# dmMaze/comic-text-detector

Hardware: AMD Instinct MI355X
Metric: pages/sec at 1024x1024 bs=32 (end-to-end detector, device-resident pages) (higher is better)
Workload: dtype f16

## Files before the change

comic-text-detector_amd/csrc/host_refine.cpp:

```cpp
#include <algorithm>
#include <cmath>
#include <cstdint>
#include <cstring>

#include "../../include/ctd_hip.h"
#include "host_refine.h"
#include "np_dispatch.h"

extern "C" int ctd_topk_colors(const int64_t* hist, double* colors) {
  int lo = -1, hi = -1;
  for (int v = 0; v < 256; ++v)
    if (hist[v] > 0) {
      if (lo < 0) lo = v;
      hi = v;
    }
  double first, last;
  if (lo < 0) first = 0.0, last = 1.0;
  else first = (double)lo, last = (double)hi;
  if (first == last) first -= 0.5, last += 0.5;
  const int nb = 255;
  double edges[256];
  const double step = (last - first) / (double)nb;
  for (int i = 0; i <= nb; ++i) edges[i] = (double)i * step + first;
  edges[nb] = last;
// ... 81 lines not shown
      const double c_top = std::min(top[k] + 30, 255.0);
      const double c_bottom = c_top - 60;
      rules[k].kind = 0;
      ctd_inrange_bounds(c_bottom, c_top, &rules[k].lo, &rules[k].hi);
    }
  }
  for (int ch = 0; ch < 3; ++ch) {
    for (int v = 0; v < 256; ++v) h[v] = hist4[256 * (1 + ch) + v];
    rules[3 + ch].kind = 1 + ch;
    rules[3 + ch].lo = ctd_otsu_from_hist(h);
    rules[3 + ch].hi = 0;
  }
}

int refine_candidates(const RRule rules[6], const uint64_t sums[6], long long npix, RCand out[4]) {
  int n = 0;
  auto pick = [&](int k) {
    RCand c;
    const unsigned long long d_pos = sums[k], d_neg = 255ull * (unsigned long long)npix - d_pos;
    c.rule = k;
    c.invert = d_neg < d_pos;
    c.dist = c.invert ? d_neg : d_pos;
    return c;
  };
  for (int k = 0; k < 3; ++k)
    if (rules[k].kind >= 0) out[n++] = pick(k);
  RCand best = pick(3);
  for (int k = 4; k < 6; ++k) {
    const RCand c = pick(k);
    if (c.dist < best.dist) best = c;
  }
  out[n++] = best;
  std::stable_sort(out, out + n, [](const RCand& a, const RCand& b) { return a.dist < b.dist; });
  return n;
}
```

comic-text-detector_amd/csrc/host_refine.h:

```cpp
#pragma once
#include <stdint.h>

struct RRule {
  int32_t kind;
  int32_t lo, hi;
};
struct RCand {
  int rule;
  int invert;
  unsigned long long dist;
};
void refine_rules(const uint32_t* hist4 , RRule rules[6]);
int refine_candidates(const RRule rules[6], const uint64_t sums[6], long long npix, RCand out[4]);
```

comic-text-detector_amd/csrc/kernels_twlds.hip:

```cpp
#include <algorithm>

#include "kernels.h"
#include "tail.h"

namespace {

constexpr int TL_MAXT = 1024;

struct Geo {
  int W, H, wp, words;
  unsigned last;
};

__device__ __forceinline__ unsigned lds_ld(const unsigned* p) {
  return __hip_atomic_load(p, __ATOMIC_RELAXED, __HIP_MEMORY_SCOPE_WORKGROUP);
}
__device__ __forceinline__ void lds_st(unsigned* p, unsigned v) {
  __hip_atomic_store(p, v, __ATOMIC_RELAXED, __HIP_MEMORY_SCOPE_WORKGROUP);
}

struct Row3 {
  unsigned prev, cur, nxt;
};
__device__ __forceinline__ Row3 row3(const unsigned* p, const Geo& g, int y, int wi) {
// ... 55 lines not shown
}
__device__ __forceinline__ void uf_union(unsigned* parent, unsigned a, unsigned b) {
  for (;;) {
    a = uf_find(parent, a);
    b = uf_find(parent, b);
    if (a == b) return;
    if (a < b) {
      const unsigned t = a;
      a = b;
      b = t;
    }
    if (atomicCAS(parent + a, a, b) == a) return;
  }
}

struct TLdsArgs {
  const TWin* wins;
  const TBand* bands;
  const int* order;
  int dilate;
  int max_words, rlay;
  int rcap;
  int* ovf;
};

__global__ __launch_bounds__(TL_MAXT) void tw_lds_kernel(TLdsArgs a) {
  extern __shared__ __attribute__((aligned(16))) unsigned lds[];
  const int t = threadIdx.x, lane = t & 63, wave = t >> 6;
  const int TL_NT = blockDim.x, NWV = TL_NT >> 6;
  const int widx = a.order[blockIdx.x];
  const TWin w = a.wins[widx];
  Geo g;
  g.W = w.w, g.H = w.h, g.wp = (w.w + 31) >> 5, g.words = g.wp * g.H;
  g.last = (w.w & 31) ? ((1u << (w.w & 31)) - 1u) : 0xffffffffu;
  const int MW = a.max_words, RL = a.rlay, RC = a.rcap;
  unsigned* const pred = lds;
  unsigned* const merged = lds + MW;
  unsigned* const cand = lds + 2 * MW;
  unsigned short* const base = (unsigned short*)(lds + 3 * MW);
  unsigned* const parent = lds + 3 * MW + ((MW + 1) >> 1);
  int* const acc = (int*)(parent + RL);
  unsigned* const red = parent + 2 * RL;
  unsigned* const tmp = parent;
  auto validw = [&](int wi) { return wi == g.wp - 1 ? g.last : 0xffffffffu; };
  const int y_t = t / g.wp, wi_t = t - y_t * g.wp;
  const int dy_t = TL_NT / g.wp, dwi_t = TL_NT - dy_t * g.wp;
  auto for_words = [&](auto&& fn) {
    int y = y_t, wi = wi_t;
    for (int i = t; i < g.words; i += TL_NT) {
      fn(i, y, wi);
      wi += dwi_t, y += dy_t;
      if (wi >= g.wp) wi -= g.wp, ++y;
    }
  };

  for_words([&](int i, int y, int wi) {
    unsigned v[8];
    load32(w.mask + (size_t)(w.y1 + y) * w.mask_w + w.x1 + 32 * wi, g.W - 32 * wi, v);
    unsigned bits = 0;
#pragma unroll
    for (int j = 0; j < 8; ++j) bits |= gt60_nibble(v[j]) << (4 * j);
    tmp[i] = bits & validw(wi);
    merged[i] = 0;
  });
  __syncthreads();
  for_words([&](int i, int y, int wi) {
    auto ext = [&](int yy, int ww) -> unsigned {
      if ((unsigned)yy >= (unsigned)g.H || (unsigned)ww >= (unsigned)g.wp) return 0xffffffffu;
      return tmp[yy * g.wp + ww] | ~validw(ww);
    };
    const unsigned cur = ext(y, wi), prev = ext(y, wi - 1), nxt = ext(y, wi + 1);
    pred[i] = cur & ((cur << 1) | (prev >> 31)) & ((cur >> 1) | (nxt << 31)) & ext(y - 1, wi) & ext(y + 1, wi) & validw(wi);
  });
  __syncthreads();

  const int seg = (g.words + TL_NT - 1) / TL_NT;
  auto starts_of = [&](int i, int wi) -> unsigned {
    const unsigned c = cand[i], cl = wi > 0 ? cand[i - 1] : 0u;
    return c & ~((c << 1) | (cl >> 31));
  };
  auto scan_runs = [&]() -> int {
    const int i0 = min(t * seg, g.words), i1 = min(i0 + seg, g.words);
    int cnt = 0;
    {
      int wi = i0 % g.wp;
      for (int i = i0; i < i1; ++i) {
        cnt += __popc(starts_of(i, wi));
        if (++wi == g.wp) wi = 0;
      }
// ... 79 lines not shown
    for_words([&](int i, int, int wi) {
      const unsigned c = cand[i];
      if (!c) return;
      const unsigned cl = wi > 0 ? cand[i - 1] : 0u;
      const unsigned sc = c & ~((c << 1) | (cl >> 31)), bc = base[i];
      unsigned add = 0;
      for_groups(c, [&](int p, unsigned grp) {
        if (acc[uf_find(parent, rid_from(bc, sc, p))] > 0) add |= grp;
      });
      if (add) merged[i] |= add;
    });
    __syncthreads();
  };
  bool overflow = false;

  for (int r = 0; r < w.nband && !overflow; ++r) {
    const TBand bd = a.bands[w.band0 + r];
    for_words([&](int i, int y, int wi) {
      const int npx = min(32, g.W - 32 * wi);
      const uint8_t* src = w.img + ((size_t)(w.y1 + y) * w.img_w + w.x1 + 32 * wi) * 3;
      unsigned v[24];
      load32(src, min(32, 3 * npx), v);
      load32(src + 32, min(32, max(0, 3 * npx - 32)), v + 8);
      load32(src + 64, min(32, max(0, 3 * npx - 64)), v + 16);
      unsigned bits = 0;
      auto byte_at = [&](int o) { return (v[o >> 2] >> (8 * (o & 3))) & 0xffu; };
      if (bd.kind == 0) {
#pragma unroll
        for (int k = 0; k < 32; ++k) {
          const int gr = gray3(byte_at(3 * k), byte_at(3 * k + 1), byte_at(3 * k + 2));
          bits |= ((gr >= bd.lo && gr <= bd.hi) ? 1u : 0u) << k;
        }
      } else {
        const int ch = bd.kind - 1;
#pragma unroll
        for (int k = 0; k < 32; ++k) {
          const unsigned c0 = byte_at(3 * k), c1 = byte_at(3 * k + 1), c2 = byte_at(3 * k + 2);
          bits |= (((int)(ch == 0 ? c0 : (ch == 1 ? c1 : c2)) > bd.lo) ? 1u : 0u) << k;
        }
      }
      if (bd.invert) bits = ~bits;
      tmp[i] = bits & validw(wi);
    });
    __syncthreads();
    for_words([&](int i, int y, int wi) {
      const Row3 c0 = row3(tmp, g, y, wi);
      unsigned out = c0.cur;
      if (out) {
        const Row3 m1 = row3(tmp, g, y - 1, wi), p1 = row3(tmp, g, y + 1, wi), m2 = row3(tmp, g, y - 2, wi), p2 = row3(tmp, g, y + 2, wi);
        const unsigned up = ring3(m1), dn = ring3(p1), cur = c0.cur;
        const unsigned single = cur & ~(shk<-1>(c0) | shk<1>(c0) | up | dn);
        const unsigned hl = cur & shk<1>(c0) & ~(shk<-1>(c0) | shk<2>(c0) | up | dn | shk<2>(m1) | shk<2>(p1));
        const unsigned hr = cur & shk<-1>(c0) & ~(shk<-2>(c0) | shk<1>(c0) | up | dn | shk<-2>(m1) | shk<-2>(p1));
        const unsigned vt = cur & p1.cur & ~(shk<-1>(c0) | shk<1>(c0) | shk<-1>(p1) | shk<1>(p1) | up | ring3(p2));
        const unsigned vb = cur & m1.cur & ~(shk<-1>(c0) | shk<1>(c0) | shk<-1>(m1) | shk<1>(m1) | dn | ring3(m2));
        out = cur & ~(single | hl | hr | vt | vb);
      }
      cand[i] = out;
// ... 103 lines not shown
      if ((unsigned)v2) atomicOr(ap, (unsigned)v2);
      if ((unsigned)(v2 >> 32)) atomicOr(ap + 1, (unsigned)(v2 >> 32));
    }
  });
}

}

size_t tw_lds_bytes(int max_words, int rcap) {
  const int rlay = std::max(rcap, (max_words + 1) / 2);
  return ((size_t)3 * max_words + (max_words + 1) / 2 + (size_t)2 * rlay + 20) * 4;
}

int tw_lds_rcap(int max_words) { return std::min(65000, std::max(1024, (int)((long long)max_words * g_tw_lds_runs_x10 / 10))); }

bool launch_tw_lds(const TWin* wins, const TBand* bands, const int* order, int n, int max_words, int rcap, int dilate, int* ovf,
                   hipStream_t st, TwLdsLaunch* used) {
  if (n <= 0) return true;
  TLdsArgs a;
  a.wins = wins, a.bands = bands, a.order = order, a.dilate = dilate, a.max_words = max_words;
  a.rcap = std::min(rcap, 65000), a.rlay = std::max(a.rcap, (max_words + 1) / 2);
  a.ovf = ovf;
  const size_t bytes = tw_lds_bytes(max_words, a.rcap);
  const int nt = g_tw_lds_threads >= 1024 ? 1024 : (g_tw_lds_threads >= 512 ? 512 : 256);
  if (used) *used = TwLdsLaunch{n, max_words, a.rcap, nt, (int)bytes, 0};
  if (bytes > 48 * 1024 &&
      hipFuncSetAttribute((const void*)tw_lds_kernel, hipFuncAttributeMaxDynamicSharedMemorySize, (int)bytes) != hipSuccess) {
    (void)hipGetLastError();
    if (used) used->refused = 1;
    return false;
  }
  hipLaunchKernelGGL(tw_lds_kernel, dim3(n), dim3(nt), bytes, st, a);
  return true;
}
```

comic-text-detector_amd/csrc/tail.h:

```cpp
#pragma once
#include "ctd_common.h"
#include "tuning.h"

struct DbcTables {
  int B, H, W, cap, rcap;
  const float* prob;
  long long prob_stride;
  const int* lab;
  const int* n_f;
  const int* n_b;
  const int* st_f;
  const int* st_b;
  const int* first_f;
  const int* first_b;
  int* par_f;
  int* par_b;
  int* off_f;
  int* off_b;
  int* hdr;
  int* row_lo;
  int* row_hi;
  double* sum_f;
  double* sum_b;
  double* ring_sum;
// ... 32 lines not shown
void launch_tw_accept_all(const TWin* wins, const TBand* bands, int n, const int* labels, int canvas_w, const int* stats,
                          int max_labels, int min_box, uint8_t* merged, int merged_w, unsigned* counters, hipStream_t st);
void launch_tw_dilate(const TWin* wins, int n, int max_pix, const uint8_t* in, uint8_t* out, uint8_t* comp, int merged_w,
                      unsigned* count255, int dilate, hipStream_t st);
void launch_tw_holes(const TWin* wins, int n, int max_pix, const int* labels2, const int* stats2, const int* first2,
                     int max_labels, const unsigned* count255, int* top2, uint8_t* merged, int merged_w,
                     unsigned* counters2, hipStream_t st);
void launch_tw_holes_all(const TWin* wins, int n, const int* labels2, const int* stats2, const int* first2, int max_labels,
                         const unsigned* count255, uint8_t* merged, int merged_w, unsigned* counters2, hipStream_t st);
void launch_tw_commit(const TWin* wins, int n, int max_pix, const uint8_t* merged, int merged_w, hipStream_t st);
size_t tw_lds_bytes(int max_words, int rcap);
int tw_lds_rcap(int max_words);
struct TwLdsLaunch {
  int n, max_words, rcap, threads, bytes, refused;
};
bool launch_tw_lds(const TWin* wins, const TBand* bands, const int* order, int n, int max_words, int rcap, int dilate, int* ovf,
                   hipStream_t st, TwLdsLaunch* used = nullptr);
void launch_mask_clear_where(uint8_t* mask, const uint8_t* refined, long long n, int thr, hipStream_t st);
void launch_copy2d_u8(const uint8_t* src, int spitch, uint8_t* dst, int dpitch, int rows, int cols, hipStream_t st);

struct MSeg {
  void* dst;
  const void* src;
  unsigned long long row_bytes;
  long long dpitch, spitch;
  int rows;
  int fill;
  int vec;
  int pad_;
};
constexpr int kMSegMax = 24;
struct MSegs {
// ... 6 lines not shown
```

comic-text-detector_amd/csrc/tail.hip:

```cpp
#include <algorithm>
#include <atomic>
#include <chrono>
#include <mutex>
#include <cmath>
#include <cstring>
#include <string>
#include <thread>
#include <vector>

#include "host_refine.h"
#include "kernels.h"
#include "tail.h"

int ctd_fail_msg(int code, const std::string& msg);

#define T_TRY(expr)                                                                                  \
  do {                                                                                               \
    hipError_t e_ = (expr);                                                                          \
    if (e_ != hipSuccess) return ctd_fail_msg(CTD_ERR_HIP, std::string(#expr) + ": " + hipGetErrorString(e_)); \
  } while (0)

namespace {

struct DevBuf {
// ... 184 lines not shown
}

static_assert(sizeof(ctd_trace_win) == 4312, "ctd_trace_win is read as a packed record (comic-text-detector_amd/tail.py)");
struct DbTrace {
  int32_t hdr[4] = {0, 0, 0, 0};
  int nf = 0, nb = 0, nr = 0;
  std::vector<int32_t> i32;
  std::vector<double> f64;
};

struct ctd_tail {
  int device = 0;
  hipStream_t st = nullptr;
  DevBuf d_dets, d_nms_ws, d_lab_f, d_ccl_ws, d_ccl_small, d_dbc_i, d_dbc_d, d_rows, d_pmask, d_refined;
  DevBuf d_wins, d_rules, d_bands, d_hist, d_sums, d_canvas, d_clab, d_cstats, d_cnt, d_merged, d_mlab, d_mstats, d_cnt2, d_small, d_crop;
  DevBuf d_wins_c, d_bands_c, d_lds;
  PinBuf h_dets, h_hdr, h_tab, h_pmask, h_refined, h_hist, h_sums, h_wins, h_rules, h_bands, h_small, h_lab;
  PinBuf h_wins_c, h_bands_c, h_lds;
  int B = 0;
  std::vector<ctd_tail_page> pages;
  std::vector<size_t> poff;
  std::vector<uint8_t*> hmask;
  size_t ptotal = 0;
  std::vector<PageOut> out;
  double ms_stage[10] = {0, 0, 0, 0, 0, 0, 0, 0, 0, 0};
  double ms_db_wait = 0;
  double ms_sub[5] = {0, 0, 0, 0, 0};
  int host_threads = 8;
  int n_lds = 0, n_canvas = 0, n_ovf = 0;
  long long lds_per_block = 64 << 10;
  double ms_lds_wait = 0;
  bool trace = false;
  std::vector<ctd_trace_win> tr_wins;
// ... 125 lines not shown
  launch_tw_dilate(dw, n, max_pix, merged_a, merged_b, comp, pm.W, count255, refine_mode == 0 ? 1 : 0, st);
  GET(t->d_mlab, mpx * 4, int, mlab);
  GET(t->d_mstats, (size_t)cap2 * 6 * 4, int, mstats);
  int* mfirst = mstats + (size_t)cap2 * 5;
  launch_ccl(comp, 1, pm.H, pm.W, 0, 8, mlab, n_dev, mstats, cap2, ws, st, 0, mfirst, 1);
  launch_label_counters_zero(counters2, n_dev, cap2, st);
  if (fused) launch_tw_holes_all(dw, n, mlab, mstats, mfirst, cap2, count255, merged_b, pm.W, counters2, st);
  else launch_tw_holes(dw, n, max_pix, mlab, mstats, mfirst, cap2, count255, top2, merged_b, pm.W, counters2, st);
  launch_tw_commit(dw, n, max_pix, merged_b, pm.W, st);
  T_TRY(chain.end());
  T_TRY(hipGetLastError());
  return CTD_OK;
}

void trace_windows(ctd_tail* t, const std::vector<WinReq>& reqs, int pass, const uint32_t* hhist, const RRule* hrules,
                   const uint64_t* hsums, const std::vector<int>& canvas_win, const std::vector<int>& again) {
  const size_t base = t->tr_wins.size();
  t->tr_wins.resize(base + reqs.size());
  for (size_t i = 0; i < reqs.size(); ++i) {
    ctd_trace_win& r = t->tr_wins[base + i];
    std::memset(&r, 0, sizeof(r));
    r.page = reqs[i].page, r.x1 = reqs[i].x1, r.y1 = reqs[i].y1, r.w = reqs[i].x2 - reqs[i].x1, r.h = reqs[i].y2 - reqs[i].y1;
    r.pass = pass, r.path = 0;
    std::memcpy(r.hist, hhist + i * 1024, sizeof(r.hist));
    for (int k = 0; k < 6; ++k) {
      const RRule& rl = hrules[i * 6 + k];
      r.rules[3 * k] = rl.kind, r.rules[3 * k + 1] = rl.lo, r.rules[3 * k + 2] = rl.hi;
      r.sums[k] = hsums[i * 6 + k];
    }
    RCand c[4];
    r.n_cand = refine_candidates(hrules + i * 6, hsums + i * 6, (long long)r.w * r.h, c);
    for (int k = 0; k < r.n_cand; ++k) r.cand_rule[k] = c[k].rule, r.cand_invert[k] = c[k].invert, r.cand_dist[k] = c[k].dist;
  }
  for (int i : canvas_win) t->tr_wins[base + i].path = 1;
  for (int i : again) t->tr_wins[base + i].path = 2;
}

int refine_windows(ctd_tail* t, const std::vector<WinReq>& reqs, int refine_mode, int pass) {
  const int n = (int)reqs.size();
  if (n == 0) return CTD_OK;
  hipStream_t st = t->st;
  GET(t->d_pmask, 0, uint8_t, pmask);
  GET(t->d_refined, 0, uint8_t, refined);
  std::vector<int> ww(n), wh(n);
  int max_pix = 1;
  for (int i = 0; i < n; ++i) {
    ww[i] = reqs[i].x2 - reqs[i].x1, wh[i] = reqs[i].y2 - reqs[i].y1;
// ... 2 lines not shown
  GET(t->h_wins, sizeof(TWin) * n, TWin, hw);
  for (int i = 0; i < n; ++i) {
    const ctd_tail_page& pg = t->pages[reqs[i].page];
    TWin& w = hw[i];
    w.img = pg.img_dev;
    w.mask = pmask + t->poff[reqs[i].page];
    w.out = refined + t->poff[reqs[i].page];
    w.img_w = pg.im_w, w.mask_w = pg.im_w, w.out_w = pg.im_w;
    w.x1 = reqs[i].x1, w.y1 = reqs[i].y1, w.w = ww[i], w.h = wh[i];
    w.mx = 0, w.my = 0;
    w.band0 = 0, w.nband = 0;
  }
  GET(t->d_wins, sizeof(TWin) * n, TWin, dw);
  GET(t->d_hist, (size_t)n * 1024 * 4, unsigned, dhist);
  GET(t->h_hist, (size_t)n * 1024 * 4, uint32_t, hhist);
  GET(t->d_sums, (size_t)n * 6 * 8, unsigned long long, dsums);
  GET(t->h_sums, (size_t)n * 6 * 8, uint64_t, hsums);
  Batch bt(st);
  T_TRY(bt.h2d(dw, hw, sizeof(TWin) * n));
  bt.fill(dhist, 0, (size_t)n * 1024 * 4);
  bt.fill(dsums, 0, (size_t)n * 6 * 8);
  bt.flush();
  launch_tw_hist(dw, n, max_pix, dhist, st);
  T_TRY(bt.d2h(hhist, dhist, (size_t)n * 1024 * 4));
  bt.flush();
  const double tr0 = now_ms();
  T_TRY(hipStreamSynchronize(st));
  const double tr1 = now_ms();
  GET(t->h_rules, sizeof(RRule) * 6 * n, RRule, hrules);
  parallel_for(n, t->host_threads, [&](int i) { refine_rules(hhist + (size_t)i * 1024, hrules + (size_t)i * 6); });
  static_assert(sizeof(RRule) == sizeof(TRule), "rule layouts must agree");
  GET(t->d_rules, sizeof(TRule) * 6 * n, TRule, drules);
  T_TRY(bt.h2d(drules, hrules, sizeof(TRule) * 6 * n));
  bt.flush();
  launch_tw_xor(dw, drules, n, max_pix, dsums, st);
  T_TRY(bt.d2h(hsums, dsums, (size_t)n * 6 * 8));
  bt.flush();
  const double tr2 = now_ms();
  T_TRY(hipStreamSynchronize(st));
  const double tr3 = now_ms();
  std::vector<TBand> bands;
  for (int i = 0; i < n; ++i) {
    RCand c[4];
    const int nc = refine_candidates(hrules + (size_t)i * 6, hsums + (size_t)i * 6, (long long)ww[i] * wh[i], c);
    hw[i].band0 = (int)bands.size(), hw[i].nband = nc;
    for (int r = 0; r < nc; ++r) {
      const RRule& rl = hrules[(size_t)i * 6 + c[r].rule];
      TBand b;
      b.win = i, b.cx = b.cy = 0, b.kind = rl.kind, b.lo = rl.lo, b.hi = rl.hi, b.invert = c[r].invert, b.round = r;
      bands.push_back(b);
    }
  }
  const int nbands = (int)bands.size();
  const long long lds_max = std::min(g_tail_lds_max_bytes, t->lds_per_block - 2048);
  std::vector<int> lds_win, canvas_win;
  std::vector<int> words(n);
  for (int i = 0; i < n; ++i) {
    words[i] = ((ww[i] + 31) >> 5) * wh[i];
    const int rc = g_tail_lds_rcap > 0 ? g_tail_lds_rcap : tw_lds_rcap(words[i]);
    if (g_tail_lds && (long long)tw_lds_bytes(words[i], std::max(rc, (words[i] + 1) / 2)) <= lds_max) lds_win.push_back(i);
    else canvas_win.push_back(i);
  }
  int nl = (int)lds_win.size();
  int* hovf = nullptr;
  if (nl) {
    std::stable_sort(lds_win.begin(), lds_win.end(), [&](int a, int b) { return words[a] < words[b]; });
    GET(t->h_bands, sizeof(TBand) * std::max(nbands, 1), TBand, hb);
    std::memcpy(hb, bands.data(), sizeof(TBand) * nbands);
    GET(t->d_bands, sizeof(TBand) * std::max(nbands, 1), TBand, db);
    GET(t->h_lds, (size_t)n * 8, int, hl);
    GET(t->d_lds, (size_t)n * 8, int, dl);
    std::memcpy(hl, lds_win.data(), sizeof(int) * nl);
    hovf = hl + n;
    T_TRY(bt.h2d(db, hb, sizeof(TBand) * nbands));
    T_TRY(bt.h2d(dw, hw, sizeof(TWin) * n));
    T_TRY(bt.h2d(dl, hl, sizeof(int) * nl));
    bt.fill(dl + n, 0, sizeof(int) * n);
    bt.flush();
    const long long cls[3] = {g_tail_lds_cls0, g_tail_lds_cls1, lds_max};
    std::vector<int> refused;
    int k0 = 0;
    for (int c = 0; c < 3 && k0 < nl; ++c) {
      int k1 = k0;
      auto need = [&](int k) {
        const int wd = words[lds_win[k]];
        const int rc = g_tail_lds_rcap > 0 ? g_tail_lds_rcap : tw_lds_rcap(wd);
        return (long long)tw_lds_bytes(wd, std::max(rc, (wd + 1) / 2));
      };
      while (k1 < nl && (c == 2 || need(k1) <= cls[c])) ++k1;
      if (k1 > k0) {
        const int mw = words[lds_win[k1 - 1]];
        TwLdsLaunch used{};
        if (!launch_tw_lds(dw, db, dl + k0, k1 - k0, mw, g_tail_lds_rcap > 0 ? g_tail_lds_rcap : tw_lds_rcap(mw),
                           refine_mode == 0 ? 1 : 0, dl + n, st, t->trace ? &used : nullptr))
          for (int k = k0; k < k1; ++k) refused.push_back(lds_win[k]);
        if (t->trace) t->tr_lds.push_back(used);
      }
      k0 = k1;
    }
    T_TRY(bt.d2h(hovf, dl + n, sizeof(int) * n));
    bt.flush();
    if (!refused.empty()) {
      std::sort(refused.begin(), refused.end());
      canvas_win.insert(canvas_win.end(), refused.begin(), refused.end());
      std::sort(canvas_win.begin(), canvas_win.end());
      std::vector<int> kept;
      for (int i : lds_win)
        if (!std::binary_search(refused.begin(), refused.end(), i)) kept.push_back(i);
      lds_win.swap(kept);
      nl = (int)lds_win.size();
    }
  }
  if (int rc = refine_canvas(t, hw, bands, canvas_win, refine_mode)) return rc;
  const double tr4 = now_ms();
  double tr5 = tr4;
  std::vector<int> again;
  if (nl) {
    T_TRY(hipStreamSynchronize(st));
    tr5 = now_ms();
    for (int k = 0; k < nl; ++k)
      if (hovf[lds_win[k]]) again.push_back(lds_win[k]);
    std::sort(again.begin(), again.end());
    t->n_lds += nl - (int)again.size(), t->n_canvas += (int)canvas_win.size() + (int)again.size(), t->n_ovf += (int)again.size();
    if (int rc = refine_canvas(t, hw, bands, again, refine_mode)) return rc;
  } else {
    t->n_canvas += (int)canvas_win.size();
  }
  T_TRY(hipGetLastError());
  if (t->trace) trace_windows(t, reqs, pass, hhist, hrules, hsums, canvas_win, again);
  t->ms_stage[4] += tr1 - tr0;
  t->ms_stage[5] += tr3 - tr2;
  t->ms_stage[6] += (now_ms() - tr5) + (tr4 - tr3) + (tr2 - tr1);
  t->ms_lds_wait += tr5 - tr4;
  return CTD_OK;
}

int layout_pages(ctd_tail* t, int B, const ctd_tail_page* pages) {
  t->B = B;
  t->pages.assign(pages, pages + B);
  t->poff.resize(B);
  size_t off = 0;
  for (int b = 0; b < B; ++b) {
    if (pages[b].im_h < 1 || pages[b].im_w < 1) return ctd_fail_msg(CTD_ERR_INVALID, "bad page size");
    t->poff[b] = off;
// ... 372 lines not shown
  if (hipDeviceGetAttribute(&smem, hipDeviceAttributeMaxSharedMemoryPerBlock, device) == hipSuccess && smem > 0) t->lds_per_block = smem;
  *out = t;
  return CTD_OK;
}

void ctd_tail_destroy(ctd_tail* t) {
  if (!t) return;
  (void)hipSetDevice(t->device);
  if (t->st) {
    (void)hipStreamSynchronize(t->st);
    (void)hipStreamDestroy(t->st);
  }
  DevBuf* dv[] = {&t->d_dets, &t->d_nms_ws, &t->d_lab_f, &t->d_ccl_ws, &t->d_ccl_small, &t->d_dbc_i, &t->d_dbc_d,
                  &t->d_rows, &t->d_pmask, &t->d_refined, &t->d_wins, &t->d_rules, &t->d_bands, &t->d_hist, &t->d_sums,
                  &t->d_canvas, &t->d_clab, &t->d_cstats, &t->d_cnt, &t->d_merged, &t->d_mlab, &t->d_mstats, &t->d_cnt2,
                  &t->d_small, &t->d_crop, &t->d_wins_c, &t->d_bands_c, &t->d_lds};
  for (DevBuf* d : dv) d->release();
  PinBuf* pv[] = {&t->h_dets, &t->h_hdr, &t->h_tab, &t->h_pmask, &t->h_refined, &t->h_hist, &t->h_sums, &t->h_wins,
                  &t->h_rules, &t->h_bands, &t->h_small, &t->h_lab, &t->h_wins_c, &t->h_bands_c, &t->h_lds};
  for (PinBuf* p : pv) p->release();
  delete t;
}

void* ctd_tail_stream(ctd_tail* t) { return t ? (void*)t->st : nullptr; }

static int drained(ctd_tail* t, int rc) {
  if (rc != CTD_OK && t && t->st) (void)hipStreamSynchronize(t->st);
  return rc;
}

static int tail_run_impl(ctd_tail* t, int32_t B, int32_t Hn, int32_t Wn, const float* blks_dev, int32_t rows, int32_t no,
                         const uint8_t* mask_u8_dev, const float* prob_dev, int64_t prob_stride, const uint8_t* bitmap_dev,
                         const ctd_tail_page* pages, const ctd_tail_params* prm, uint8_t* const* mask_out,
                         uint8_t* const* refined_out, void* ready_event) {
// ... 404 lines not shown
```

Before: 3255.

## Fuse refine-rule sums and candidate selection into the LDS window kernel

Result: no change. 3276 (median of 6 runs) (+0.6%).

```diff
diff --git a/comic-text-detector_amd/csrc/host_refine.cpp b/comic-text-detector_amd/csrc/host_refine.cpp
--- a/comic-text-detector_amd/csrc/host_refine.cpp
+++ b/comic-text-detector_amd/csrc/host_refine.cpp
@@ -119,23 +119,8 @@
 }
 
 int refine_candidates(const RRule rules[6], const uint64_t sums[6], long long npix, RCand out[4]) {
-  int n = 0;
-  auto pick = [&](int k) {
-    RCand c;
-    const unsigned long long d_pos = sums[k], d_neg = 255ull * (unsigned long long)npix - d_pos;
-    c.rule = k;
-    c.invert = d_neg < d_pos;
-    c.dist = c.invert ? d_neg : d_pos;
-    return c;
-  };
+  unsigned valid3 = 0;
   for (int k = 0; k < 3; ++k)
-    if (rules[k].kind >= 0) out[n++] = pick(k);
-  RCand best = pick(3);
-  for (int k = 4; k < 6; ++k) {
-    const RCand c = pick(k);
-    if (c.dist < best.dist) best = c;
-  }
-  out[n++] = best;
-  std::stable_sort(out, out + n, [](const RCand& a, const RCand& b) { return a.dist < b.dist; });
-  return n;
+    if (rules[k].kind >= 0) valid3 |= 1u << k;
+  return refine_decide(valid3, sums, npix, out);
 }
diff --git a/comic-text-detector_amd/csrc/host_refine.h b/comic-text-detector_amd/csrc/host_refine.h
--- a/comic-text-detector_amd/csrc/host_refine.h
+++ b/comic-text-detector_amd/csrc/host_refine.h
@@ -1,14 +1,7 @@
 #pragma once
 #include <stdint.h>
 
-struct RRule {
-  int32_t kind;
-  int32_t lo, hi;
-};
-struct RCand {
-  int rule;
-  int invert;
-  unsigned long long dist;
-};
+#include "refine_decide.h"
+
 void refine_rules(const uint32_t* hist4 , RRule rules[6]);
 int refine_candidates(const RRule rules[6], const uint64_t sums[6], long long npix, RCand out[4]);
diff --git a/comic-text-detector_amd/csrc/kernels_twlds.hip b/comic-text-detector_amd/csrc/kernels_twlds.hip
--- a/comic-text-detector_amd/csrc/kernels_twlds.hip
+++ b/comic-text-detector_amd/csrc/kernels_twlds.hip
@@ -1,6 +1,10 @@
 #include <algorithm>
 
+#include <mutex>
+#include <type_traits>
+
 #include "kernels.h"
+#include "refine_decide.h"
 #include "tail.h"
 
 namespace {
@@ -93,16 +97,48 @@
   }
 }
 
+template <int From, int To, class F>
+__device__ __forceinline__ void static_for(F&& f) {
+  if constexpr (From < To) {
+    f(std::integral_constant<int, From>{});
+    static_for<From + 1, To>(f);
+  }
+}
+
 struct TLdsArgs {
   const TWin* wins;
   const TBand* bands;
+  const TRule* rules;
   const int* order;
   int dilate;
   int max_words, rlay;
   int rcap;
   int* ovf;
+  unsigned long long* sums;
+  unsigned* cword;
 };
 
+struct GeK {
+  unsigned add, nd, en;
+};
+__device__ __forceinline__ GeK ge_const(int d) {
+  d = min(max(d, 0), 256);
+  GeK k;
+  k.en = d > 255 ? 0u : 0x80808080u;
+  k.add = (0x80u - (unsigned)(d & 0x7f)) * 0x01010101u;
+  k.nd = (d & 0x80) ? 0u : 0xffffffffu;
+  return k;
+}
+__device__ __forceinline__ unsigned ge4(unsigned x, const GeK& k) {
+  const unsigned t = (x & 0x7f7f7f7fu) + k.add;
+  return ((x & t) | ((x | t) & k.nd)) & k.en;
+}
+__device__ __forceinline__ unsigned gather4(unsigned w0, unsigned w1, unsigned w2, unsigned w3, int s) {
+  const unsigned sel = 0x0c0c0000u | ((4u + (unsigned)s) << 8) | (unsigned)s;
+  return __builtin_amdgcn_perm(w1, w0, sel) | (__builtin_amdgcn_perm(w3, w2, sel) << 16);
+}
+
+template <int WPT>
 __global__ __launch_bounds__(TL_MAXT) void tw_lds_kernel(TLdsArgs a) {
   extern __shared__ __attribute__((aligned(16))) unsigned lds[];
   const int t = threadIdx.x, lane = t & 63, wave = t >> 6;
@@ -132,17 +168,110 @@
       if (wi >= g.wp) wi -= g.wp, ++y;
     }
   };
-
-  for_words([&](int i, int y, int wi) {
-    unsigned v[8];
-    load32(w.mask + (size_t)(w.y1 + y) * w.mask_w + w.x1 + 32 * wi, g.W - 32 * wi, v);
-    unsigned bits = 0;
-#pragma unroll
-    for (int j = 0; j < 8; ++j) bits |= gt60_nibble(v[j]) << (4 * j);
-    tmp[i] = bits & validw(wi);
-    merged[i] = 0;
-  });
-  __syncthreads();
+  auto for_owned = [&](auto&& fn) {
+    int y = y_t, wi = wi_t;
+    static_for<0, WPT>([&](auto jc) {
+      const int i = t + decltype(jc)::value * TL_NT;
+      if (i < g.words) fn(jc, i, y, wi);
+      wi += dwi_t, y += dy_t;
+      if (wi >= g.wp) wi -= g.wp, ++y;
+    });
+  };
+  unsigned pl[WPT > 0 ? WPT : 1][6];
+  unsigned cw = 0;
+
+  if constexpr (WPT == 0) {
+    for_words([&](int i, int y, int wi) {
+      unsigned v[8];
+      load32(w.mask + (size_t)(w.y1 + y) * w.mask_w + w.x1 + 32 * wi, g.W - 32 * wi, v);
+      unsigned bits = 0;
+#pragma unroll
+      for (int j = 0; j < 8; ++j) bits |= gt60_nibble(v[j]) << (4 * j);
+      tmp[i] = bits & validw(wi);
+      merged[i] = 0;
+    });
+    __syncthreads();
+  } else {
+    GeK glo[3], ghi[3], gch[3];
+    int chn[3];
+    unsigned valid3 = 0, used6 = 0;
+#pragma unroll
+    for (int k = 0; k < 3; ++k) {
+      const TRule rg = a.rules[(size_t)widx * 6 + k], rc = a.rules[(size_t)widx * 6 + 3 + k];
+      const bool on = rg.kind == 0;
+      glo[k] = ge_const(on ? rg.lo : 256);
+      ghi[k] = ge_const(min(rg.hi, 255) + 1);
+      gch[k] = ge_const(rc.kind >= 1 ? min(rc.lo, 255) + 1 : 256);
+      chn[k] = rc.kind;
+      valid3 |= (rg.kind >= 0 ? 1u : 0u) << k;
+      used6 |= ((rg.kind >= 0 ? 1u : 0u) << k) | ((rc.kind >= 0 ? 1u : 0u) << (3 + k));
+    }
+    if (t < 13) red[t] = 0u;
+    unsigned cnt[6] = {0, 0, 0, 0, 0, 0}, msum[6] = {0, 0, 0, 0, 0, 0}, mall = 0;
+#pragma unroll
+    for (int j = 0; j < WPT; ++j)
+#pragma unroll
+      for (int k = 0; k < 6; ++k) pl[j][k] = 0u;
+    for_owned([&](auto jc, int i, int y, int wi) {
+      constexpr int j = decltype(jc)::value;
+      const int npx = min(32, g.W - 32 * wi);
+      const uint8_t* src = w.img + ((size_t)(w.y1 + y) * w.img_w + w.x1 + 32 * wi) * 3;
+      unsigned v[24], mv[8];
+      load32(w.mask + (size_t)(w.y1 + y) * w.mask_w + w.x1 + 32 * wi, npx, mv);
+      load32(src, min(32, 3 * npx), v);
+      load32(src + 32, min(32, max(0, 3 * npx - 32)), v + 8);
+      load32(src + 64, min(32, max(0, 3 * npx - 64)), v + 16);
+      unsigned bits = 0;
+#pragma unroll
+      for (int q = 0; q < 8; ++q) {
+        bits |= gt60_nibble(mv[q]) << (4 * q);
+        mall = __builtin_amdgcn_sad_u8(mv[q], 0u, mall);
+      }
+      tmp[i] = bits & validw(wi);
+      merged[i] = 0;
+      unsigned p6[6] = {0, 0, 0, 0, 0, 0};
+#pragma unroll
+      for (int q = 0; q < 8; ++q) {
+        const unsigned m4 = gather4(mv[q >> 2], mv[2 + (q >> 2)], mv[4 + (q >> 2)], mv[6 + (q >> 2)], q & 3);
+        unsigned c4[3];
+#pragma unroll
+        for (int c = 0; c < 3; ++c) {
+          const int o = 3 * q + c;
+          c4[c] = gather4(v[o >> 2], v[6 + (o >> 2)], v[12 + (o >> 2)], v[18 + (o >> 2)], o & 3);
+        }
+        unsigned y4 = 0;
+#pragma unroll
+        for (int k = 0; k < 4; ++k)
+          y4 |= (unsigned)gray3((c4[0] >> (8 * k)) & 0xffu, (c4[1] >> (8 * k)) & 0xffu, (c4[2] >> (8 * k)) & 0xffu) << (8 * k);
+#pragma unroll
+        for (int k = 0; k < 6; ++k) {
+          unsigned on;
+          if (k < 3) {
+            on = ge4(y4, glo[k]) & ~ge4(y4, ghi[k]);
+          } else {
+            const int ch = chn[k - 3];
+            on = ge4(ch == 1 ? c4[0] : (ch == 2 ? c4[1] : c4[2]), gch[k - 3]);
+          }
+          p6[k] |= on >> (7 - q);
+          msum[k] = __builtin_amdgcn_sad_u8(m4 & (on | (on - (on >> 7))), 0u, msum[k]);
+        }
+      }
+      const unsigned vw = validw(wi);
+#pragma unroll
+      for (int k = 0; k < 6; ++k) {
+        pl[j][k] = p6[k];
+        cnt[k] += (unsigned)__popc(p6[k] & vw);
+      }
+    });
+    __syncthreads();
+#pragma unroll
+    for (int k = 0; k < 13; ++k) {
+      unsigned x = k < 6 ? cnt[k] : (k < 12 ? msum[k - 6] : mall);
+      for (int off = 32; off > 0; off >>= 1) x += __shfl_down(x, off);
+      if (lane == 0 && x) atomicAdd(red + k, x);
+    }
+    cw = valid3 | (used6 << 8);
+  }
   for_words([&](int i, int y, int wi) {
     auto ext = [&](int yy, int ww) -> unsigned {
       if ((unsigned)yy >= (unsigned)g.H || (unsigned)ww >= (unsigned)g.wp) return 0xffffffffu;
@@ -152,6 +281,22 @@
     pred[i] = cur & ((cur << 1) | (prev >> 31)) & ((cur >> 1) | (nxt << 31)) & ext(y - 1, wi) & ext(y + 1, wi) & validw(wi);
   });
   __syncthreads();
+  if constexpr (WPT > 0) {
+    const unsigned valid3 = cw & 7u, used6 = cw >> 8;
+    const unsigned long long M = red[12];
+    uint64_t sums[6];
+#pragma unroll
+    for (int k = 0; k < 6; ++k)
+      sums[k] = ((used6 >> k) & 1u) ? 255ull * red[k] + M - 2ull * red[6 + k] : 0ull;
+    RCand cs[4];
+    const int nc = refine_decide(valid3, sums, (long long)g.W * g.H, cs);
+    cw = refine_pack(nc, cs);
+    if (t == 0) {
+#pragma unroll
+      for (int k = 0; k < 6; ++k) a.sums[(size_t)widx * 6 + k] = sums[k];
+      a.cword[widx] = cw;
+    }
+  }
 
   const int seg = (g.words + TL_NT - 1) / TL_NT;
   auto starts_of = [&](int i, int wi) -> unsigned {
@@ -261,34 +406,50 @@
   };
   bool overflow = false;
 
-  for (int r = 0; r < w.nband && !overflow; ++r) {
-    const TBand bd = a.bands[w.band0 + r];
-    for_words([&](int i, int y, int wi) {
-      const int npx = min(32, g.W - 32 * wi);
-      const uint8_t* src = w.img + ((size_t)(w.y1 + y) * w.img_w + w.x1 + 32 * wi) * 3;
-      unsigned v[24];
-      load32(src, min(32, 3 * npx), v);
-      load32(src + 32, min(32, max(0, 3 * npx - 32)), v + 8);
-      load32(src + 64, min(32, max(0, 3 * npx - 64)), v + 16);
-      unsigned bits = 0;
-      auto byte_at = [&](int o) { return (v[o >> 2] >> (8 * (o & 3))) & 0xffu; };
-      if (bd.kind == 0) {
-#pragma unroll
-        for (int k = 0; k < 32; ++k) {
-          const int gr = gray3(byte_at(3 * k), byte_at(3 * k + 1), byte_at(3 * k + 2));
-          bits |= ((gr >= bd.lo && gr <= bd.hi) ? 1u : 0u) << k;
+  const int nround = WPT > 0 ? refine_word_count(cw) : w.nband;
+  for (int r = 0; r < nround && !overflow; ++r) {
+    if constexpr (WPT > 0) {
+      const int rule = refine_word_rule(cw, r);
+      const unsigned inv = refine_word_invert(cw, r) ? 0xffffffffu : 0u;
+      unsigned pick[6];
+#pragma unroll
+      for (int k = 0; k < 6; ++k) pick[k] = rule == k ? 0xffffffffu : 0u;
+      for_owned([&](auto jc, int i, int, int wi) {
+        constexpr int j = decltype(jc)::value;
+        unsigned bits = 0;
+#pragma unroll
+        for (int k = 0; k < 6; ++k) bits |= pl[j][k] & pick[k];
+        tmp[i] = (bits ^ inv) & validw(wi);
+      });
+    } else {
+      const TBand bd = a.bands[w.band0 + r];
+      for_words([&](int i, int y, int wi) {
+        const int npx = min(32, g.W - 32 * wi);
+        const uint8_t* src = w.img + ((size_t)(w.y1 + y) * w.img_w + w.x1 + 32 * wi) * 3;
+        unsigned v[24];
+        load32(src, min(32, 3 * npx), v);
+        load32(src + 32, min(32, max(0, 3 * npx - 32)), v + 8);
+        load32(src + 64, min(32, max(0, 3 * npx - 64)), v + 16);
+        unsigned bits = 0;
+        auto byte_at = [&](int o) { return (v[o >> 2] >> (8 * (o & 3))) & 0xffu; };
+        if (bd.kind == 0) {
+#pragma unroll
+          for (int k = 0; k < 32; ++k) {
+            const int gr = gray3(byte_at(3 * k), byte_at(3 * k + 1), byte_at(3 * k + 2));
+            bits |= ((gr >= bd.lo && gr <= bd.hi) ? 1u : 0u) << k;
+          }
+        } else {
+          const int ch = bd.kind - 1;
+#pragma unroll
+          for (int k = 0; k < 32; ++k) {
+            const unsigned c0 = byte_at(3 * k), c1 = byte_at(3 * k + 1), c2 = byte_at(3 * k + 2);
+            bits |= (((int)(ch == 0 ? c0 : (ch == 1 ? c1 : c2)) > bd.lo) ? 1u : 0u) << k;
+          }
         }
-      } else {
-        const int ch = bd.kind - 1;
-#pragma unroll
-        for (int k = 0; k < 32; ++k) {
-          const unsigned c0 = byte_at(3 * k), c1 = byte_at(3 * k + 1), c2 = byte_at(3 * k + 2);
-          bits |= (((int)(ch == 0 ? c0 : (ch == 1 ? c1 : c2)) > bd.lo) ? 1u : 0u) << k;
-        }
-      }
-      if (bd.invert) bits = ~bits;
-      tmp[i] = bits & validw(wi);
-    });
+        if (bd.invert) bits = ~bits;
+        tmp[i] = bits & validw(wi);
+      });
+    }
     __syncthreads();
     for_words([&](int i, int y, int wi) {
       const Row3 c0 = row3(tmp, g, y, wi);
@@ -422,22 +583,59 @@
 
 int tw_lds_rcap(int max_words) { return std::min(65000, std::max(1024, (int)((long long)max_words * g_tw_lds_runs_x10 / 10))); }
 
-bool launch_tw_lds(const TWin* wins, const TBand* bands, const int* order, int n, int max_words, int rcap, int dilate, int* ovf,
-                   hipStream_t st, TwLdsLaunch* used) {
+namespace {
+
+int tw_lds_threads() { return g_tw_lds_threads >= 1024 ? 1024 : (g_tw_lds_threads >= 512 ? 512 : 256); }
+
+constexpr int kLdsDevices = 64;
+template <int WPT>
+hipError_t lds_limit_once() {
+  static std::once_flag once[kLdsDevices];
+  static hipError_t err[kLdsDevices];
+  int dev = 0;
+  if (hipError_t e = hipGetDevice(&dev)) return e;
+  if (dev < 0 || dev >= kLdsDevices) return hipErrorInvalidDevice;
+  std::call_once(once[dev], [&] {
+    int lim = 0;
+    hipError_t e = hipDeviceGetAttribute(&lim, hipDeviceAttributeMaxSharedMemoryPerBlock, dev);
+    if (e == hipSuccess) e = hipFuncSetAttribute((const void*)tw_lds_kernel<WPT>, hipFuncAttributeMaxDynamicSharedMemorySize, lim);
+    err[dev] = e;
+  });
+  return err[dev];
+}
+
+template <int WPT>
+bool launch_one(const TLdsArgs& a, int n, int nt, size_t bytes, hipStream_t st) {
+  if (bytes > 48 * 1024 && lds_limit_once<WPT>() != hipSuccess) {
+    (void)hipGetLastError();
+    return false;
+  }
+  hipLaunchKernelGGL(tw_lds_kernel<WPT>, dim3(n), dim3(nt), bytes, st, a);
+  return hipGetLastError() == hipSuccess;
+}
+
+}
+
+int tw_lds_cached_wpt(int max_words) {
+  const int need = (max_words + tw_lds_threads() - 1) / tw_lds_threads();
+  return need <= 4 ? 4 : (need <= 7 ? 7 : 0);
+}
+
+bool launch_tw_lds(const TWin* wins, const TBand* bands, const TRule* rules, const int* order, int n, int max_words, int rcap,
+                   int dilate, int* ovf, unsigned long long* sums, unsigned* cword, hipStream_t st, TwLdsLaunch* used) {
   if (n <= 0) return true;
   TLdsArgs a;
-  a.wins = wins, a.bands = bands, a.order = order, a.dilate = dilate, a.max_words = max_words;
+  a.wins = wins, a.bands = bands, a.rules = rules, a.order = order, a.dilate = dilate, a.max_words = max_words;
   a.rcap = std::min(rcap, 65000), a.rlay = std::max(a.rcap, (max_words + 1) / 2);
-  a.ovf = ovf;
+  a.ovf = ovf, a.sums = sums, a.cword = cword;
   const size_t bytes = tw_lds_bytes(max_words, a.rcap);
-  const int nt = g_tw_lds_threads >= 1024 ? 1024 : (g_tw_lds_threads >= 512 ? 512 : 256);
+  const int nt = tw_lds_threads();
   if (used) *used = TwLdsLaunch{n, max_words, a.rcap, nt, (int)bytes, 0};
-  if (bytes > 48 * 1024 &&
-      hipFuncSetAttribute((const void*)tw_lds_kernel, hipFuncAttributeMaxDynamicSharedMemorySize, (int)bytes) != hipSuccess) {
-    (void)hipGetLastError();
-    if (used) used->refused = 1;
-    return false;
-  }
-  hipLaunchKernelGGL(tw_lds_kernel, dim3(n), dim3(nt), bytes, st, a);
-  return true;
-}
+  const int wpt = bands ? 0 : tw_lds_cached_wpt(max_words);
+  bool ok = false;
+  if (bands) ok = launch_one<0>(a, n, nt, bytes, st);
+  else if (wpt == 4) ok = launch_one<4>(a, n, nt, bytes, st);
+  else if (wpt == 7) ok = launch_one<7>(a, n, nt, bytes, st);
+  if (!ok && used) used->refused = 1;
+  return ok;
+}
diff --git a/comic-text-detector_amd/csrc/refine_decide.h b/comic-text-detector_amd/csrc/refine_decide.h
--- /dev/null
+++ b/comic-text-detector_amd/csrc/refine_decide.h
@@ -0,0 +1,65 @@
+#pragma once
+#include <stdint.h>
+
+#if defined(__HIPCC__) || defined(__CUDACC__)
+#define CTD_HD __host__ __device__
+#else
+#define CTD_HD
+#endif
+
+struct RRule {
+  int32_t kind;
+  int32_t lo, hi;
+};
+struct RCand {
+  int rule;
+  int invert;
+  unsigned long long dist;
+};
+
+CTD_HD inline int refine_decide(unsigned valid3, const uint64_t sums[6], long long npix, RCand out[4]) {
+  const unsigned long long full = 255ull * (unsigned long long)npix;
+  unsigned long long key[4];
+  for (int k = 0; k < 3; ++k) {
+    const unsigned long long d_pos = sums[k], d_neg = full - d_pos;
+    out[k].rule = k;
+    out[k].invert = d_neg < d_pos;
+    out[k].dist = out[k].invert ? d_neg : d_pos;
+    key[k] = ((valid3 >> k) & 1u) ? out[k].dist : ~0ull;
+  }
+  out[3].rule = 3, out[3].invert = 0, out[3].dist = ~0ull;
+  for (int k = 3; k < 6; ++k) {
+    const unsigned long long d_pos = sums[k], d_neg = full - d_pos;
+    const int inv = d_neg < d_pos;
+    const unsigned long long d = inv ? d_neg : d_pos;
+    if (k == 3 || d < out[3].dist) out[3].rule = k, out[3].invert = inv, out[3].dist = d;
+  }
+  key[3] = out[3].dist;
+#if defined(__HIP_DEVICE_COMPILE__)
+#pragma unroll
+#endif
+  for (int i = 1; i < 4; ++i) {
+#if defined(__HIP_DEVICE_COMPILE__)
+#pragma unroll
+#endif
+    for (int j = i; j > 0; --j) {
+      if (key[j] < key[j - 1]) {
+        const unsigned long long tk = key[j];
+        key[j] = key[j - 1], key[j - 1] = tk;
+        const RCand tc = out[j];
+        out[j] = out[j - 1], out[j - 1] = tc;
+      }
+    }
+  }
+  return 1 + (int)(valid3 & 1u) + (int)((valid3 >> 1) & 1u) + (int)((valid3 >> 2) & 1u);
+}
+
+CTD_HD inline unsigned refine_pack(int n, const RCand c[4]) {
+  unsigned w = (unsigned)n;
+  for (int r = 0; r < 4; ++r)
+    if (r < n) w |= ((unsigned)c[r].rule | ((unsigned)c[r].invert << 3)) << (4 + 4 * r);
+  return w;
+}
+CTD_HD inline int refine_word_count(unsigned w) { return (int)(w & 7u); }
+CTD_HD inline int refine_word_rule(unsigned w, int r) { return (int)((w >> (4 + 4 * r)) & 7u); }
+CTD_HD inline int refine_word_invert(unsigned w, int r) { return (int)((w >> (7 + 4 * r)) & 1u); }
diff --git a/comic-text-detector_amd/csrc/tail.h b/comic-text-detector_amd/csrc/tail.h
--- a/comic-text-detector_amd/csrc/tail.h
+++ b/comic-text-detector_amd/csrc/tail.h
@@ -70,8 +70,9 @@
 struct TwLdsLaunch {
   int n, max_words, rcap, threads, bytes, refused;
 };
-bool launch_tw_lds(const TWin* wins, const TBand* bands, const int* order, int n, int max_words, int rcap, int dilate, int* ovf,
-                   hipStream_t st, TwLdsLaunch* used = nullptr);
+int tw_lds_cached_wpt(int max_words);
+bool launch_tw_lds(const TWin* wins, const TBand* bands, const TRule* rules, const int* order, int n, int max_words, int rcap,
+                   int dilate, int* ovf, unsigned long long* sums, unsigned* cword, hipStream_t st, TwLdsLaunch* used = nullptr);
 void launch_mask_clear_where(uint8_t* mask, const uint8_t* refined, long long n, int thr, hipStream_t st);
 void launch_copy2d_u8(const uint8_t* src, int spitch, uint8_t* dst, int dpitch, int rows, int cols, hipStream_t st);
 
diff --git a/comic-text-detector_amd/csrc/tail.hip b/comic-text-detector_amd/csrc/tail.hip
--- a/comic-text-detector_amd/csrc/tail.hip
+++ b/comic-text-detector_amd/csrc/tail.hip
@@ -222,9 +222,9 @@
   hipStream_t st = nullptr;
   DevBuf d_dets, d_nms_ws, d_lab_f, d_ccl_ws, d_ccl_small, d_dbc_i, d_dbc_d, d_rows, d_pmask, d_refined;
   DevBuf d_wins, d_rules, d_bands, d_hist, d_sums, d_canvas, d_clab, d_cstats, d_cnt, d_merged, d_mlab, d_mstats, d_cnt2, d_small, d_crop;
-  DevBuf d_wins_c, d_bands_c, d_lds;
+  DevBuf d_wins_c, d_bands_c, d_lds, d_xor;
   PinBuf h_dets, h_hdr, h_tab, h_pmask, h_refined, h_hist, h_sums, h_wins, h_rules, h_bands, h_small, h_lab;
-  PinBuf h_wins_c, h_bands_c, h_lds;
+  PinBuf h_wins_c, h_bands_c, h_lds, h_xor;
   int B = 0;
   std::vector<ctd_tail_page> pages;
   std::vector<size_t> poff;
@@ -380,7 +380,8 @@
 }
 
 void trace_windows(ctd_tail* t, const std::vector<WinReq>& reqs, int pass, const uint32_t* hhist, const RRule* hrules,
-                   const uint64_t* hsums, const std::vector<int>& canvas_win, const std::vector<int>& again) {
+                   const uint64_t* hsums, const std::vector<unsigned>& cwords, const std::vector<int>& canvas_win,
+                   const std::vector<int>& again) {
   const size_t base = t->tr_wins.size();
   t->tr_wins.resize(base + reqs.size());
   for (size_t i = 0; i < reqs.size(); ++i) {
@@ -394,9 +395,12 @@
       r.rules[3 * k] = rl.kind, r.rules[3 * k + 1] = rl.lo, r.rules[3 * k + 2] = rl.hi;
       r.sums[k] = hsums[i * 6 + k];
     }
-    RCand c[4];
-    r.n_cand = refine_candidates(hrules + i * 6, hsums + i * 6, (long long)r.w * r.h, c);
-    for (int k = 0; k < r.n_cand; ++k) r.cand_rule[k] = c[k].rule, r.cand_invert[k] = c[k].invert, r.cand_dist[k] = c[k].dist;
+    const unsigned long long full = 255ull * (unsigned long long)((long long)r.w * r.h);
+    r.n_cand = refine_word_count(cwords[i]);
+    for (int k = 0; k < r.n_cand && k < 4; ++k) {
+      r.cand_rule[k] = refine_word_rule(cwords[i], k), r.cand_invert[k] = refine_word_invert(cwords[i], k);
+      r.cand_dist[k] = r.cand_invert[k] ? full - r.sums[r.cand_rule[k]] : r.sums[r.cand_rule[k]];
+    }
   }
   for (int i : canvas_win) t->tr_wins[base + i].path = 1;
   for (int i : again) t->tr_wins[base + i].path = 2;
@@ -429,44 +433,19 @@
   GET(t->d_wins, sizeof(TWin) * n, TWin, dw);
   GET(t->d_hist, (size_t)n * 1024 * 4, unsigned, dhist);
   GET(t->h_hist, (size_t)n * 1024 * 4, uint32_t, hhist);
-  GET(t->d_sums, (size_t)n * 6 * 8, unsigned long long, dsums);
-  GET(t->h_sums, (size_t)n * 6 * 8, uint64_t, hsums);
+  GET(t->d_sums, (size_t)n * 12 * 8, unsigned long long, dsums);
+  GET(t->h_sums, (size_t)n * 12 * 8, uint64_t, hsums);
+  GET(t->h_lds, (size_t)n * 12, int, hl);
+  GET(t->d_lds, (size_t)n * 12, int, dl);
   Batch bt(st);
   T_TRY(bt.h2d(dw, hw, sizeof(TWin) * n));
   bt.fill(dhist, 0, (size_t)n * 1024 * 4);
-  bt.fill(dsums, 0, (size_t)n * 6 * 8);
+  bt.fill(dsums, 0, (size_t)n * 12 * 8);
+  bt.fill(dl + n, 0, sizeof(int) * 2 * n);
   bt.flush();
   launch_tw_hist(dw, n, max_pix, dhist, st);
   T_TRY(bt.d2h(hhist, dhist, (size_t)n * 1024 * 4));
   bt.flush();
-  const double tr0 = now_ms();
-  T_TRY(hipStreamSynchronize(st));
-  const double tr1 = now_ms();
-  GET(t->h_rules, sizeof(RRule) * 6 * n, RRule, hrules);
-  parallel_for(n, t->host_threads, [&](int i) { refine_rules(hhist + (size_t)i * 1024, hrules + (size_t)i * 6); });
-  static_assert(sizeof(RRule) == sizeof(TRule), "rule layouts must agree");
-  GET(t->d_rules, sizeof(TRule) * 6 * n, TRule, drules);
-  T_TRY(bt.h2d(drules, hrules, sizeof(TRule) * 6 * n));
-  bt.flush();
-  launch_tw_xor(dw, drules, n, max_pix, dsums, st);
-  T_TRY(bt.d2h(hsums, dsums, (size_t)n * 6 * 8));
-  bt.flush();
-  const double tr2 = now_ms();
-  T_TRY(hipStreamSynchronize(st));
-  const double tr3 = now_ms();
-  std::vector<TBand> bands;
-  for (int i = 0; i < n; ++i) {
-    RCand c[4];
-    const int nc = refine_candidates(hrules + (size_t)i * 6, hsums + (size_t)i * 6, (long long)ww[i] * wh[i], c);
-    hw[i].band0 = (int)bands.size(), hw[i].nband = nc;
-    for (int r = 0; r < nc; ++r) {
-      const RRule& rl = hrules[(size_t)i * 6 + c[r].rule];
-      TBand b;
-      b.win = i, b.cx = b.cy = 0, b.kind = rl.kind, b.lo = rl.lo, b.hi = rl.hi, b.invert = c[r].invert, b.round = r;
-      bands.push_back(b);
-    }
-  }
-  const int nbands = (int)bands.size();
   const long long lds_max = std::min(g_tail_lds_max_bytes, t->lds_per_block - 2048);
   std::vector<int> lds_win, canvas_win;
   std::vector<int> words(n);
@@ -477,23 +456,13 @@
     else canvas_win.push_back(i);
   }
   int nl = (int)lds_win.size();
-  int* hovf = nullptr;
-  if (nl) {
-    std::stable_sort(lds_win.begin(), lds_win.end(), [&](int a, int b) { return words[a] < words[b]; });
-    GET(t->h_bands, sizeof(TBand) * std::max(nbands, 1), TBand, hb);
-    std::memcpy(hb, bands.data(), sizeof(TBand) * nbands);
-    GET(t->d_bands, sizeof(TBand) * std::max(nbands, 1), TBand, db);
-    GET(t->h_lds, (size_t)n * 8, int, hl);
-    GET(t->d_lds, (size_t)n * 8, int, dl);
-    std::memcpy(hl, lds_win.data(), sizeof(int) * nl);
-    hovf = hl + n;
-    T_TRY(bt.h2d(db, hb, sizeof(TBand) * nbands));
-    T_TRY(bt.h2d(dw, hw, sizeof(TWin) * n));
-    T_TRY(bt.h2d(dl, hl, sizeof(int) * nl));
-    bt.fill(dl + n, 0, sizeof(int) * n);
-    bt.flush();
+  std::stable_sort(lds_win.begin(), lds_win.end(), [&](int a, int b) { return words[a] < words[b]; });
+  struct Launch {
+    int k0, k1, mw;
+  };
+  std::vector<Launch> cached, banded;
+  {
     const long long cls[3] = {g_tail_lds_cls0, g_tail_lds_cls1, lds_max};
-    std::vector<int> refused;
     int k0 = 0;
     for (int c = 0; c < 3 && k0 < nl; ++c) {
       int k1 = k0;
@@ -505,26 +474,99 @@
       while (k1 < nl && (c == 2 || need(k1) <= cls[c])) ++k1;
       if (k1 > k0) {
         const int mw = words[lds_win[k1 - 1]];
-        TwLdsLaunch used{};
-        if (!launch_tw_lds(dw, db, dl + k0, k1 - k0, mw, g_tail_lds_rcap > 0 ? g_tail_lds_rcap : tw_lds_rcap(mw),
-                           refine_mode == 0 ? 1 : 0, dl + n, st, t->trace ? &used : nullptr))
-          for (int k = k0; k < k1; ++k) refused.push_back(lds_win[k]);
-        if (t->trace) t->tr_lds.push_back(used);
+        (tw_lds_cached_wpt(mw) > 0 ? cached : banded).push_back(Launch{k0, k1, mw});
       }
       k0 = k1;
     }
-    T_TRY(bt.d2h(hovf, dl + n, sizeof(int) * n));
+  }
+  const double tr0 = now_ms();
+  T_TRY(hipStreamSynchronize(st));
+  const double tr1 = now_ms();
+  GET(t->h_rules, sizeof(RRule) * 6 * n, RRule, hrules);
+  parallel_for(n, t->host_threads, [&](int i) { refine_rules(hhist + (size_t)i * 1024, hrules + (size_t)i * 6); });
+  static_assert(sizeof(RRule) == sizeof(TRule), "rule layouts must agree");
+  GET(t->d_rules, sizeof(TRule) * 6 * n, TRule, drules);
+  T_TRY(bt.h2d(drules, hrules, sizeof(TRule) * 6 * n));
+  if (nl) {
+    std::memcpy(hl, lds_win.data(), sizeof(int) * nl);
+    T_TRY(bt.h2d(dl, hl, sizeof(int) * nl));
+  }
+  bt.flush();
+  std::vector<int> refused;
+  auto launch = [&](const Launch& L, const TBand* db) {
+    TwLdsLaunch used{};
+    if (!launch_tw_lds(dw, db, drules, dl + L.k0, L.k1 - L.k0, L.mw, g_tail_lds_rcap > 0 ? g_tail_lds_rcap : tw_lds_rcap(L.mw),
+                       refine_mode == 0 ? 1 : 0, dl + n, dsums, (unsigned*)(dl + 2 * n), st, t->trace ? &used : nullptr))
+      for (int k = L.k0; k < L.k1; ++k) refused.push_back(lds_win[k]);
+    if (t->trace) t->tr_lds.push_back(used);
+  };
+  for (const Launch& L : cached) launch(L, nullptr);
+  std::vector<int> old_win(canvas_win);
+  for (const Launch& L : banded)
+    for (int k = L.k0; k < L.k1; ++k) old_win.push_back(lds_win[k]);
+  old_win.insert(old_win.end(), refused.begin(), refused.end());
+  std::sort(old_win.begin(), old_win.end());
+  std::vector<unsigned> cwords(n, 0u);
+  std::vector<TBand> bands;
+  auto add_bands = [&](int i, const uint64_t* sums) {
+    RCand c[4];
+    const int nc = refine_candidates(hrules + (size_t)i * 6, sums, (long long)ww[i] * wh[i], c);
+    hw[i].band0 = (int)bands.size(), hw[i].nband = nc;
+    for (int r = 0; r < nc; ++r) {
+      const RRule& rl = hrules[(size_t)i * 6 + c[r].rule];
+      TBand b;
+      b.win = i, b.cx = b.cy = 0, b.kind = rl.kind, b.lo = rl.lo, b.hi = rl.hi, b.invert = c[r].invert, b.round = r;
+      bands.push_back(b);
+    }
+    cwords[i] = refine_pack(nc, c);
+  };
+  const int m = (int)old_win.size();
+  uint64_t* const xsums = hsums + (size_t)n * 6;
+  double tr2 = now_ms(), tr3 = tr2;
+  if (m) {
+    GET(t->h_xor, (sizeof(TWin) + sizeof(TRule) * 6) * m, TWin, hxw);
+    GET(t->d_xor, (sizeof(TWin) + sizeof(TRule) * 6) * m, TWin, dxw);
+    TRule* const hxr = (TRule*)(hxw + m);
+    int old_pix = 1;
+    for (int j = 0; j < m; ++j) {
+      hxw[j] = hw[old_win[j]];
+      std::memcpy(hxr + (size_t)j * 6, hrules + (size_t)old_win[j] * 6, sizeof(TRule) * 6);
+      old_pix = std::max(old_pix, ww[old_win[j]] * wh[old_win[j]]);
+    }
+    T_TRY(bt.h2d(dxw, hxw, (sizeof(TWin) + sizeof(TRule) * 6) * m));
     bt.flush();
-    if (!refused.empty()) {
-      std::sort(refused.begin(), refused.end());
-      canvas_win.insert(canvas_win.end(), refused.begin(), refused.end());
-      std::sort(canvas_win.begin(), canvas_win.end());
-      std::vector<int> kept;
-      for (int i : lds_win)
-        if (!std::binary_search(refused.begin(), refused.end(), i)) kept.push_back(i);
-      lds_win.swap(kept);
-      nl = (int)lds_win.size();
-    }
+    launch_tw_xor(dxw, (const TRule*)(dxw + m), m, old_pix, dsums + (size_t)n * 6, st);
+    T_TRY(bt.d2h(xsums, dsums + (size_t)n * 6, (size_t)m * 6 * 8));
+    bt.flush();
+    tr2 = now_ms();
+    T_TRY(hipStreamSynchronize(st));
+    tr3 = now_ms();
+    for (int j = 0; j < m; ++j) add_bands(old_win[j], xsums + (size_t)j * 6);
+    if (!banded.empty()) {
+      const int nbands = (int)bands.size();
+      GET(t->h_bands, sizeof(TBand) * std::max(nbands, 1), TBand, hb);
+      std::memcpy(hb, bands.data(), sizeof(TBand) * nbands);
+      GET(t->d_bands, sizeof(TBand) * std::max(nbands, 1), TBand, db);
+      T_TRY(bt.h2d(db, hb, sizeof(TBand) * nbands));
+      T_TRY(bt.h2d(dw, hw, sizeof(TWin) * n));
+      bt.flush();
+      for (const Launch& L : banded) launch(L, db);
+    }
+  }
+  if (!refused.empty()) {
+    std::sort(refused.begin(), refused.end());
+    canvas_win.insert(canvas_win.end(), refused.begin(), refused.end());
+    std::sort(canvas_win.begin(), canvas_win.end());
+    std::vector<int> kept;
+    for (int i : lds_win)
+      if (!std::binary_search(refused.begin(), refused.end(), i)) kept.push_back(i);
+    lds_win.swap(kept);
+    nl = (int)lds_win.size();
+  }
+  if (nl) {
+    T_TRY(bt.d2h(hl + n, dl + n, sizeof(int) * 2 * n));
+    T_TRY(bt.d2h(hsums, dsums, (size_t)n * 6 * 8));
+    bt.flush();
   }
   if (int rc = refine_canvas(t, hw, bands, canvas_win, refine_mode)) return rc;
   const double tr4 = now_ms();
@@ -533,8 +575,19 @@
   if (nl) {
     T_TRY(hipStreamSynchronize(st));
     tr5 = now_ms();
-    for (int k = 0; k < nl; ++k)
-      if (hovf[lds_win[k]]) again.push_back(lds_win[k]);
+  }
+  for (int j = 0; j < m; ++j) std::memcpy(hsums + (size_t)old_win[j] * 6, xsums + (size_t)j * 6, 6 * 8);
+  if (nl) {
+    const int* hovf = hl + n;
+    std::vector<char> is_old(n, 0);
+    for (int i : old_win) is_old[i] = 1;
+    for (int k = 0; k < nl; ++k) {
+      const int i = lds_win[k];
+      if (!is_old[i]) cwords[i] = (unsigned)hl[2 * n + i];
+      if (!hovf[i]) continue;
+      again.push_back(i);
+      if (!is_old[i]) add_bands(i, hsums + (size_t)i * 6);
+    }
     std::sort(again.begin(), again.end());
     t->n_lds += nl - (int)again.size(), t->n_canvas += (int)canvas_win.size() + (int)again.size(), t->n_ovf += (int)again.size();
     if (int rc = refine_canvas(t, hw, bands, again, refine_mode)) return rc;
@@ -542,7 +595,7 @@
     t->n_canvas += (int)canvas_win.size();
   }
   T_TRY(hipGetLastError());
-  if (t->trace) trace_windows(t, reqs, pass, hhist, hrules, hsums, canvas_win, again);
+  if (t->trace) trace_windows(t, reqs, pass, hhist, hrules, hsums, cwords, canvas_win, again);
   t->ms_stage[4] += tr1 - tr0;
   t->ms_stage[5] += tr3 - tr2;
   t->ms_stage[6] += (now_ms() - tr5) + (tr4 - tr3) + (tr2 - tr1);
@@ -945,10 +998,10 @@
   DevBuf* dv[] = {&t->d_dets, &t->d_nms_ws, &t->d_lab_f, &t->d_ccl_ws, &t->d_ccl_small, &t->d_dbc_i, &t->d_dbc_d,
                   &t->d_rows, &t->d_pmask, &t->d_refined, &t->d_wins, &t->d_rules, &t->d_bands, &t->d_hist, &t->d_sums,
                   &t->d_canvas, &t->d_clab, &t->d_cstats, &t->d_cnt, &t->d_merged, &t->d_mlab, &t->d_mstats, &t->d_cnt2,
-                  &t->d_small, &t->d_crop, &t->d_wins_c, &t->d_bands_c, &t->d_lds};
+                  &t->d_small, &t->d_crop, &t->d_wins_c, &t->d_bands_c, &t->d_lds, &t->d_xor};
   for (DevBuf* d : dv) d->release();
   PinBuf* pv[] = {&t->h_dets, &t->h_hdr, &t->h_tab, &t->h_pmask, &t->h_refined, &t->h_hist, &t->h_sums, &t->h_wins,
-                  &t->h_rules, &t->h_bands, &t->h_small, &t->h_lab, &t->h_wins_c, &t->h_bands_c, &t->h_lds};
+                  &t->h_rules, &t->h_bands, &t->h_small, &t->h_lab, &t->h_wins_c, &t->h_bands_c, &t->h_lds, &t->h_xor};
   for (PinBuf* p : pv) p->release();
   delete t;
 }
```
